# ototoi/pbrt-r3

Measured on AMD Instinct MI355X. Metric: Mrays/s, higher is better.
Workload: dtype f32

## Files before the change

### pbrt-r3_amd/csrc/pt_kernels.hip

```cpp
#include <hip/hip_runtime.h>
#include <cstdlib>
#include "pt_device.h"
#include "pt_device_math.h"
#include "pt_bxdf.h"
#include "pt_sphere.h"
#include "pt_texture.h"
#include <type_traits>
#include "pt_lobes.h"
#include "pt_kernels.h"
#include "../../include/pbrtgpu.h"

#ifndef PT_SHADE_PF_DEEP
#define PT_SHADE_PF_DEEP 0
#endif
#ifndef PT_LOBES_IN_LDS
#define PT_LOBES_IN_LDS 1
#endif
#ifndef PT_TEX_PROGS_GLOBAL
#define PT_TEX_PROGS_GLOBAL 1
#endif
#ifndef PT_LIGHTS_IN_LDS
#define PT_LIGHTS_IN_LDS 8
#endif
#ifndef PT_TEX_NOUNROLL
// ... 799 lines not shown
        "v_add_u32 %[sa], %[slot], %[sa]\n\t"
        "v_mov_b32 %[top], %[c0]\n\t"
        "ds_write_b32 %[sa], %[c0]\n\t"
        "s_mov_b64 exec, %[e1]\n\t"
        "v_add_u32 %[sa], %[slot], %[sa]\n\t"
        "v_mov_b32 %[top], %[c1]\n\t"
        "ds_write_b32 %[sa], %[c1]\n\t"
        "s_mov_b64 exec, %[e2]\n\t"
        "v_add_u32 %[sa], %[slot], %[sa]\n\t"
        "v_mov_b32 %[top], %[c2]\n\t"
        "ds_write_b32 %[sa], %[c2]\n\t"
        "s_mov_b64 exec, %[e3]\n\t"
        "v_add_u32 %[sa], %[slot], %[sa]\n\t"
        "v_mov_b32 %[top], %[c3]\n\t"
        "ds_write_b32 %[sa], %[c3]\n\t"
        "s_mov_b64 exec, %[sv]"
        : [sa] "+v"(sa), [top] "+v"(top), [sv] "=&s"(sv)
        : [e0] "s"(e0), [e1] "s"(e1), [e2] "s"(e2), [e3] "s"(e3), [c0] "v"(c0), [c1] "v"(c1), [c2] "v"(c2), [c3] "v"(c3), [slot] "s"(PT_SLOT)
        : "memory");
}
typedef __attribute__((address_space(3))) void* pt_lds_void;
typedef const __attribute__((address_space(1))) void* pt_global_cvoid;
typedef float pt_v4f __attribute__((ext_vector_type(4)));
typedef uint32_t pt_v4u __attribute__((ext_vector_type(4)));
PT_DEV float4 lds_load4(uint32_t a) { const pt_v4f v = *(__attribute__((address_space(3))) const pt_v4f*)(size_t)a; return make_float4(v.x, v.y, v.z, v.w); }
PT_DEV uint4 lds_load4u(uint32_t a) { const pt_v4u v = *(__attribute__((address_space(3))) const pt_v4u*)(size_t)a; return make_uint4(v.x, v.y, v.z, v.w); }
PT_DEV uint32_t node_round_issue(const PtScene& sc, LaneRay& r, TravCtx& c, bool w_node) {
    uint32_t ref = PT_EMPTY_REF, top = PT_EMPTY_REF;
    if (w_node) {
#ifdef PT_STACK_HIST
        atomicAdd(c.spill - ((size_t)blockIdx.x * PT_BLOCK + threadIdx.x) - PT_DIAG_WORDS + 1024u + min(fs_slot(c, r.sa), 63u), 1u);
#endif
        ref = r.top;
        r.sa -= PT_SLOT;
        top = lds_load(r.sa);
        c.n_nodes++;
    }
    lds_store(c.idx_pub, ref);
    __builtin_amdgcn_fence(__ATOMIC_RELEASE, "wavefront");
    __builtin_amdgcn_wave_barrier();
    __builtin_amdgcn_fence(__ATOMIC_ACQUIRE, "wavefront");
    {
        const uint4 ia = lds_load4u(c.idx_ld), ib = lds_load4u(c.idx_ld + 16u);
        const uint32_t ids[8] = {ia.x, ia.y, ia.z, ia.w, ib.x, ib.y, ib.z, ib.w};
        const uint32_t lane = threadIdx.x & 63u;
        const uint32_t coff = ((lane & 7u) ^ (lane >> 3)) << 4;
        const char* nb = reinterpret_cast<const char*>(sc.nodes);
        const uint32_t piece0 = (uint32_t)__builtin_amdgcn_readfirstlane((int)c.stage_wave);
#pragma unroll
        for (uint32_t j = 0; j < 8u; j++)
            if (ids[j] != PT_EMPTY_REF)
                __builtin_amdgcn_global_load_lds((pt_global_cvoid)(nb + ((ids[j] << 7) + coff)), (pt_lds_void)(size_t)(piece0 + j * 1024u), 16, 0, 0);
    }
    return top;
}
PT_DEV void node_round_finish(LaneRay& r, TravCtx& c, bool w_node, uint32_t top) {
    if (w_node) {
        const float4 nx = lds_load4(r.o_nx), fx = lds_load4(r.o_fx), ny = lds_load4(r.o_ny), fy = lds_load4(r.o_fy), nz = lds_load4(r.o_nz), fz = lds_load4(r.o_fz);
        const uint4 ch = lds_load4u(c.stage_chunk(6u));
        const uint32_t lut = lds_load(c.stage_chunk(7u) + 4u);
        const float ox = r.o.x, oy = r.o.y, oz = r.o.z, ix = r.idir.x, iy = r.idir.y, iz = r.idir.z;
#define PT_SLAB(C) (v_min3(v_min(r.tmax, (fx.C - ox) * ix), (fy.C - oy) * iy, (fz.C - oz) * iz) >= v_max3(v_max(r.tmin, (nx.C - ox) * ix), (ny.C - oy) * iy, (nz.C - oz) * iz))
        const bool h0 = PT_SLAB(x), h1 = PT_SLAB(y), h2 = PT_SLAB(z), h3 = PT_SLAB(w);
#undef PT_SLAB
        const bool T = (lut & r.m_t) != 0u, L = (lut & r.m_l) != 0u, R = (lut & r.m_r) != 0u;
        const uint32_t l0 = L ? ch.x : ch.y, l1 = L ? ch.y : ch.x, r0 = R ? ch.z : ch.w, r1 = R ? ch.w : ch.z;
        const uint32_t c0 = T ? l0 : r0, c1 = T ? l1 : r1, c2 = T ? r0 : l0, c3 = T ? r1 : l1;
        const unsigned long long H0 = __ballot(h0), H1 = __ballot(h1), H2 = __ballot(h2), H3 = __ballot(h3), Tm = __ballot(T), Lm = __ballot(L), Rm = __ballot(R);
        const unsigned long long yl = Lm & (H0 ^ H1), el0 = H1 ^ yl, el1 = H0 ^ yl;
        const unsigned long long yr = Rm & (H2 ^ H3), er0 = H3 ^ yr, er1 = H2 ^ yr;
        const unsigned long long y0 = Tm & (el0 ^ er0), e0 = er0 ^ y0, e2 = el0 ^ y0;
        const unsigned long long y1 = Tm & (el1 ^ er1), e1 = er1 ^ y1, e3 = el1 ^ y1;
        fs_push4_exec(r.sa, top, c0, c1, c2, c3, e0, e1, e2, e3);
        r.top = top;
    }
}

template <int TOUCH>
PT_DEV void node_step_lean(const PtScene& sc, LaneRay& r, TravCtx& c) {
    const uint32_t ref = r.top;
    r.sa -= PT_SLOT;
    uint32_t top = lds_load(r.sa);
    c.n_nodes++;
    const char* nb = reinterpret_cast<const char*>(sc.nodes);
    const uint32_t no = ref << 7;
    float4 nx, fx, ny, fy, nz, fz;
    uint4 ch;
#if PT_TOP_NODES > 0
    const bool in_lds = no < c.top_bytes;
    c.n_nodes_lds += in_lds ? 1u : 0u;
    if (in_lds) {
        const uint32_t la = c.top_lds + no - (no >> 3);
        nx = lds_load4(la + r.o_nx); fx = lds_load4(la + r.o_fx); ny = lds_load4(la + r.o_ny); fy = lds_load4(la + r.o_fy);
        nz = lds_load4(la + r.o_nz); fz = lds_load4(la + r.o_fz);
        ch = lds_load4u(la + 96u);
    }
    if (!in_lds)
#endif
    {
        nx = *reinterpret_cast<const float4*>(nb + (no + r.o_nx)); fx = *reinterpret_cast<const float4*>(nb + (no + r.o_fx));
        ny = *reinterpret_cast<const float4*>(nb + (no + r.o_ny)); fy = *reinterpret_cast<const float4*>(nb + (no + r.o_fy));
        nz = *reinterpret_cast<const float4*>(nb + (no + r.o_nz)); fz = *reinterpret_cast<const float4*>(nb + (no + r.o_fz));
        ch = *reinterpret_cast<const uint4*>(nb + (no + 96u));
    }
    const float ox = r.o.x, oy = r.o.y, oz = r.o.z, ix = r.idir.x, iy = r.idir.y, iz = r.idir.z;
#define PT_SLAB(C) (v_min3(v_min(r.tmax, (fx.C - ox) * ix), (fy.C - oy) * iy, (fz.C - oz) * iz) >= v_max3(v_max(r.tmin, (nx.C - ox) * ix), (ny.C - oy) * iy, (nz.C - oz) * iz))
    const bool h0 = PT_SLAB(x), h1 = PT_SLAB(y), h2 = PT_SLAB(z), h3 = PT_SLAB(w);
#undef PT_SLAB
    const bool T = __builtin_amdgcn_ubfe(r.sbits, __builtin_amdgcn_ubfe(ch.x, PT_REF_AXIS_SHIFT, 2), 1) != 0u;
    const bool L = __builtin_amdgcn_ubfe(r.sbits, __builtin_amdgcn_ubfe(ch.y, PT_REF_AXIS_SHIFT, 2), 1) != 0u;
    const bool R = __builtin_amdgcn_ubfe(r.sbits, __builtin_amdgcn_ubfe(ch.w, PT_REF_AXIS_SHIFT, 2), 1) != 0u;
    const uint32_t l0 = L ? ch.x : ch.y, l1 = L ? ch.y : ch.x, r0 = R ? ch.z : ch.w, r1 = R ? ch.w : ch.z;
    const uint32_t c0 = T ? l0 : r0, c1 = T ? l1 : r1, c2 = T ? r0 : l0, c3 = T ? r1 : l1;
    const unsigned long long H0 = __ballot(h0), H1 = __ballot(h1), H2 = __ballot(h2), H3 = __ballot(h3), Tm = __ballot(T), Lm = __ballot(L), Rm = __ballot(R);
    const unsigned long long yl = Lm & (H0 ^ H1), el0 = H1 ^ yl, el1 = H0 ^ yl;
    const unsigned long long yr = Rm & (H2 ^ H3), er0 = H3 ^ yr, er1 = H2 ^ yr;
    const unsigned long long y0 = Tm & (el0 ^ er0), e0 = er0 ^ y0, e2 = el0 ^ y0;
    const unsigned long long y1 = Tm & (el1 ^ er1), e1 = er1 ^ y1, e3 = el1 ^ y1;
    fs_push4_exec(r.sa, top, c0, c1, c2, c3, e0, e1, e2, e3);
    r.top = top;
    if constexpr (TOUCH != 0) {
        unsigned long long p0, p1, p2, p3 = 0ull;
        if (TOUCH >= 4) { p0 = e0; p1 = e1; p2 = e2; p3 = e3; }
        else { p0 = e0 & (e1 | e2 | e3); p1 = e1 & (e2 | e3); p2 = e2 & e3; }
        const unsigned long long me = 1ull << (threadIdx.x & 63u);
        const char* tb = reinterpret_cast<const char*>(sc.tris);
        auto touch = [&](uint32_t cref) {
            if (TOUCH == 2 && (cref & PT_LEAF_BIT)) return;
            if (TOUCH >= 3 && !(cref & PT_LEAF_BIT)) return;
            const char* a = (cref & PT_LEAF_BIT) ? tb + (size_t)(cref & PT_LEAF_FIRST_MASK) * 48u : nb + (size_t)(cref << 7);
            uint32_t v = *reinterpret_cast<const uint32_t*>(a);
            asm volatile("" :: "v"(v));
            if (TOUCH == 5 && ((cref >> PT_LEAF_COUNT_SHIFT) & 7u) >= 2u) {
                uint32_t w = *reinterpret_cast<const uint32_t*>(a + 128);
                asm volatile("" :: "v"(w));
            }
        };
        if (p0 & me) touch(c0);
        if (p1 & me) touch(c1);
        if (p2 & me) touch(c2);
        if (p3 & me) touch(c3);
    }
}

#ifndef PT_NODE_COOP
#define PT_NODE_COOP 1
#endif
#ifndef PT_COOP_TOUCH
#define PT_COOP_TOUCH 0
#endif
#if PT_NODE_COOP
#define PT_PAIR_U(x) ((uint32_t)__builtin_amdgcn_update_dpp(0, (int)(x), 0xB1, 0xF, 0xF, false))
#define PT_PAIR_F(x) __builtin_bit_cast(float, __builtin_amdgcn_update_dpp(0, __builtin_bit_cast(int, (x)), 0xB1, 0xF, 0xF, false))
template <int TOUCH>
PT_DEV void node_step_coop(const PtScene& sc, LaneRay& r, TravCtx& c, bool w_node, unsigned long long m_node) {
    constexpr unsigned long long kEven = 0x5555555555555555ull, kOdd = 0xAAAAAAAAAAAAAAAAull;
    const unsigned long long ev = m_node & kEven, od = m_node & kOdd;
    const unsigned long long m_y = ev | (ev << 1), m_z = od | (od >> 1);
    if (__builtin_amdgcn_inverse_ballot_w64(m_y | m_z)) {
        const uint32_t ref = r.top;
        const uint32_t no = ref << 7;
        const char* nb = reinterpret_cast<const char*>(sc.nodes);
        uint32_t top = PT_EMPTY_REF;
        const bool in_lds = w_node && no < c.top_bytes;
        if (w_node) { r.sa -= PT_SLOT; top = lds_load(r.sa); c.n_nodes++; c.n_nodes_lds += in_lds ? 1u : 0u; }
        const unsigned long long m_lds = __ballot(in_lds), le = m_lds & kEven, lo = m_lds & kOdd;
        const unsigned long long y_lds = le | (le << 1), z_lds = lo | (lo >> 1);
        const uint32_t base = in_lds ? c.top_lds + no - (no >> 3) : no;
        uint32_t a1 = base + r.o_nx, a2 = base + r.o_ny, a3 = base + r.o_nz;
        uint32_t b1 = PT_PAIR_U(base + r.o_fx), b2 = PT_PAIR_U(base + r.o_fy), b3 = PT_PAIR_U(base + r.o_fz);
        unsigned long long sv;
        asm volatile("s_mov_b64 %[sv], exec\n\ts_and_b64 exec, exec, %[om]\n\tv_swap_b32 %0, %3\n\tv_swap_b32 %1, %4\n\tv_swap_b32 %2, %5\n\ts_mov_b64 exec, %[sv]"
                     : "+v"(a1), "+v"(a2), "+v"(a3), "+v"(b1), "+v"(b2), "+v"(b3), [sv] "=&s"(sv) : [om] "s"(kOdd));
        float4 x1, x2, x3, x4, x5, x6;
        uint4 ch;
        if (__builtin_amdgcn_inverse_ballot_w64(m_y & y_lds)) { x1 = lds_load4(a1); x2 = lds_load4(a2); x3 = lds_load4(a3); }
        if (__builtin_amdgcn_inverse_ballot_w64(m_z & z_lds)) { x4 = lds_load4(b1); x5 = lds_load4(b2); x6 = lds_load4(b3); }
        if (in_lds) ch = lds_load4u(base + 96u);
        if (__builtin_amdgcn_inverse_ballot_w64(m_y & ~y_lds)) {
            x1 = *reinterpret_cast<const float4*>(nb + a1); x2 = *reinterpret_cast<const float4*>(nb + a2); x3 = *reinterpret_cast<const float4*>(nb + a3);
        }
        if (__builtin_amdgcn_inverse_ballot_w64(m_z & ~z_lds)) {
            x4 = *reinterpret_cast<const float4*>(nb + b1); x5 = *reinterpret_cast<const float4*>(nb + b2); x6 = *reinterpret_cast<const float4*>(nb + b3);
        }
        if (__builtin_amdgcn_inverse_ballot_w64(m_node & ~m_lds)) ch = *reinterpret_cast<const uint4*>(nb + (no + 96u));
        asm volatile("s_mov_b64 %[sv], exec\n\ts_and_b64 exec, exec, %[om]\n\t"
                     "v_swap_b32 %0, %12\n\tv_swap_b32 %1, %13\n\tv_swap_b32 %2, %14\n\tv_swap_b32 %3, %15\n\t"
                     "v_swap_b32 %4, %16\n\tv_swap_b32 %5, %17\n\tv_swap_b32 %6, %18\n\tv_swap_b32 %7, %19\n\t"
                     "v_swap_b32 %8, %20\n\tv_swap_b32 %9, %21\n\tv_swap_b32 %10, %22\n\tv_swap_b32 %11, %23\n\t"
                     "s_mov_b64 exec, %[sv]\n\ts_nop 1"
                     : "+v"(x1.x), "+v"(x1.y), "+v"(x1.z), "+v"(x1.w), "+v"(x2.x), "+v"(x2.y), "+v"(x2.z), "+v"(x2.w), "+v"(x3.x), "+v"(x3.y), "+v"(x3.z), "+v"(x3.w),
                       "+v"(x4.x), "+v"(x4.y), "+v"(x4.z), "+v"(x4.w), "+v"(x5.x), "+v"(x5.y), "+v"(x5.z), "+v"(x5.w), "+v"(x6.x), "+v"(x6.y), "+v"(x6.z), "+v"(x6.w), [sv] "=&s"(sv)
                     : [om] "s"(kOdd));
        const float ox = r.o.x, oy = r.o.y, oz = r.o.z, ix = r.idir.x, iy = r.idir.y, iz = r.idir.z;
#define PT_SLAB(C) (v_min3(v_min(r.tmax, (PT_PAIR_F(x4.C) - ox) * ix), (PT_PAIR_F(x5.C) - oy) * iy, (PT_PAIR_F(x6.C) - oz) * iz) >= \
                    v_max3(v_max(r.tmin, (x1.C - ox) * ix), (x2.C - oy) * iy, (x3.C - oz) * iz))
        const bool h0 = PT_SLAB(x), h1 = PT_SLAB(y), h2 = PT_SLAB(z), h3 = PT_SLAB(w);
#undef PT_SLAB
        const bool T = __builtin_amdgcn_ubfe(r.sbits, __builtin_amdgcn_ubfe(ch.x, PT_REF_AXIS_SHIFT, 2), 1) != 0u;
        const bool L = __builtin_amdgcn_ubfe(r.sbits, __builtin_amdgcn_ubfe(ch.y, PT_REF_AXIS_SHIFT, 2), 1) != 0u;
        const bool R = __builtin_amdgcn_ubfe(r.sbits, __builtin_amdgcn_ubfe(ch.w, PT_REF_AXIS_SHIFT, 2), 1) != 0u;
        const uint32_t l0 = L ? ch.x : ch.y, l1 = L ? ch.y : ch.x, r0 = R ? ch.z : ch.w, r1 = R ? ch.w : ch.z;
        const uint32_t c0 = T ? l0 : r0, c1 = T ? l1 : r1, c2 = T ? r0 : l0, c3 = T ? r1 : l1;
        const unsigned long long H0 = __ballot(h0) & m_node, H1 = __ballot(h1) & m_node, H2 = __ballot(h2) & m_node, H3 = __ballot(h3) & m_node;
        const unsigned long long Tm = __ballot(T), Lm = __ballot(L), Rm = __ballot(R);
        const unsigned long long yl = Lm & (H0 ^ H1), el0 = H1 ^ yl, el1 = H0 ^ yl;
        const unsigned long long yr = Rm & (H2 ^ H3), er0 = H3 ^ yr, er1 = H2 ^ yr;
        const unsigned long long y0 = Tm & (el0 ^ er0), e0 = er0 ^ y0, e2 = el0 ^ y0;
        const unsigned long long y1 = Tm & (el1 ^ er1), e1 = er1 ^ y1, e3 = el1 ^ y1;
        fs_push4_exec(r.sa, top, c0, c1, c2, c3, e0, e1, e2, e3);
        if (w_node) r.top = top;
        if constexpr (TOUCH != 0 && PT_COOP_TOUCH) {
            const unsigned long long p0 = e0 & (e1 | e2 | e3), p1 = e1 & (e2 | e3), p2 = e2 & e3;
            const char* tb = reinterpret_cast<const char*>(sc.tris);
            auto touch = [&](uint32_t cref) {
                if (!(cref & PT_LEAF_BIT)) return;
                uint32_t v = *reinterpret_cast<const uint32_t*>(tb + (size_t)(cref & PT_LEAF_FIRST_MASK) * 48u);
                asm volatile("" :: "v"(v));
            };
            if (__builtin_amdgcn_inverse_ballot_w64(p0)) touch(c0);
            if (__builtin_amdgcn_inverse_ballot_w64(p1)) touch(c1);
            if (__builtin_amdgcn_inverse_ballot_w64(p2)) touch(c2);
        }
    }
}
#endif

template <bool SPH, bool INST, bool ALPHA = false>
PT_DEV int32_t trace_closest(const PtScene& sc, V3 o, V3 d, float t_max, TravCtx& c, float* t_out, uint32_t* inst_out) {
    LaneRay r;
    ray_begin(sc, r, o, d, t_max);
    while (!ray_done(r)) ray_step<SPH, INST, ALPHA>(sc, r, false, c);
    *t_out = r.ray_tmax;
    *inst_out = r.best_inst;
    return r.best;
}
template <bool SPH, bool INST, bool ALPHA = false>
PT_DEV bool trace_any(const PtScene& sc, V3 o, V3 d, float t_max, TravCtx& c) {
    LaneRay r;
    ray_begin(sc, r, o, d, t_max);
    while (!ray_done(r)) ray_step<SPH, INST, ALPHA>(sc, r, true, c);
    return r.best >= 0;
}

PT_DEV void flush_counters(PtCounters* g, unsigned long long* s_cnt, unsigned long long regular, unsigned long long shadow,
                           unsigned long long nodes, unsigned long long tris) {
    if (threadIdx.x < 4) s_cnt[threadIdx.x] = 0;
    __syncthreads();
    if (regular) atomicAdd(&s_cnt[0], regular);
    if (shadow) atomicAdd(&s_cnt[1], shadow);
    if (nodes) atomicAdd(&s_cnt[2], nodes);
    if (tris) atomicAdd(&s_cnt[3], tris);
    __syncthreads();
    if (threadIdx.x == 0) {
        if (s_cnt[0]) atomicAdd(&g->regular_rays, s_cnt[0]);
        if (s_cnt[1]) atomicAdd(&g->shadow_rays, s_cnt[1]);
        if (s_cnt[2]) atomicAdd(&g->nodes, s_cnt[2]);
        if (s_cnt[3]) atomicAdd(&g->tris, s_cnt[3]);
    }
}

PT_DEV uint32_t wave_ticket(uint32_t* ticket) {
    uint32_t base = 0;
    if ((threadIdx.x & 63) == 0) base = atomicAdd(ticket, 64u);
    return (uint32_t)__builtin_amdgcn_readfirstlane((int)base);
}

#ifdef PT_PROFILE_PHASES
#define PT_PROF_T(name) const unsigned long long name = (unsigned long long)__builtin_readcyclecounter()
#define PT_PROF_SET(name) name = (unsigned long long)__builtin_readcyclecounter()
#else
#define PT_PROF_T(name) do { } while (0)
#define PT_PROF_SET(name) do { } while (0)
#endif
#ifndef PT_REFILL_MIN
#define PT_REFILL_MIN 8
#endif
#ifndef PT_LEAF_MIN
#define PT_LEAF_MIN 24
#endif
#ifndef PT_LEAF_MIN_INST
#define PT_LEAF_MIN_INST 40
#endif
#ifndef PT_TRACE_WAVES
#define PT_TRACE_WAVES 4
#endif
#ifndef PT_TRACE_DIST_WAVES
#if PT_NODE_STAGED
#define PT_TRACE_DIST_WAVES 3
#else
#define PT_TRACE_DIST_WAVES 4
#endif
#endif

#ifndef PT_LEAF_TRIS_MIN
#define PT_LEAF_TRIS_MIN 56
#endif
#ifndef PT_LEAF_LANES_MIN
#define PT_LEAF_LANES_MIN 18
#endif
#ifndef PT_WALK_BATCH
#define PT_WALK_BATCH 1
#endif
#ifndef PT_SPH_LANES_MIN
#define PT_SPH_LANES_MIN 8
#endif
#ifndef PT_LEAF_TRIS_FUSED
#define PT_LEAF_TRIS_FUSED 0
#endif
template <bool DIST, bool SPH, bool INST = false, int TOUCH = 0, bool ALPHA = false>
PT_DEV void trace_body(const PtScene& sc, const PtPaths& P, const PtQueues& Q, PtCounters* cnt, uint32_t* spill, uint32_t spill_depth, uint32_t* err) {
    constexpr uint32_t TB = DIST ? PT_TBLOCK : PT_BLOCK;
    __shared__ uint32_t s_stack[(DIST ? PT_FS_SLOTS : PT_LDS_STACK) * TB];
    __shared__ unsigned long long s_cnt[4];
#if PT_NODE_STAGED
    __shared__ __attribute__((aligned(16))) unsigned char s_stage[DIST ? (PT_BLOCK / 64) * 8192 : 16];
    __shared__ uint32_t s_idx[DIST ? PT_BLOCK + PT_BLOCK / 4 : 1];
    float4* const s_res = reinterpret_cast<float4*>(s_stage + (threadIdx.x >> 6) * 8192u) - (threadIdx.x & ~63u);
    unsigned char* const s_map = reinterpret_cast<unsigned char*>(&s_idx[(threadIdx.x >> 6) * 80u + 64u]) - (threadIdx.x & ~63u);
#else
    __shared__ float4 s_res[DIST ? TB : 1];
    __shared__ unsigned char s_map[DIST ? TB : 1];
#endif
#if PT_TOP_NODES > 0 && !PT_NODE_STAGED
    __shared__ float4 s_top[DIST ? PT_TOP_NODES * 7 : 1];
#endif
    TravCtx c;
    c.lds = &s_stack[threadIdx.x];
    c.top_lds = 0; c.top_bytes = 0; c.n_nodes_lds = 0;
    c.spill_stride = gridDim.x * TB;
    c.spill = spill + PT_DIAG_WORDS + (size_t)blockIdx.x * TB + threadIdx.x;
    c.spill_depth = spill_depth;
    c.n_nodes = 0; c.n_tris = 0; c.overflow = 0;
    c.lane_base = 0; c.stage_wave = 0; c.stage_own = 0; c.idx_pub = 0; c.idx_ld = 0;
    if constexpr (DIST) {
        s_stack[threadIdx.x] = PT_EMPTY_REF;
        c.lane_base = lds_addr_of(&s_stack[threadIdx.x]);
#if PT_NODE_STAGED
        const uint32_t ln = threadIdx.x & 63u, wv = threadIdx.x >> 6;
        c.stage_wave = lds_addr_of(reinterpret_cast<const uint32_t*>(s_stage + wv * 8192u));
        c.stage_own = c.stage_wave + (ln >> 3) * 1024u + (ln & 7u) * 128u;
        c.idx_pub = lds_addr_of(&s_idx[wv * 80u + (ln & 7u) * 8u + (ln >> 3)]);
        c.idx_ld = lds_addr_of(&s_idx[wv * 80u + (ln >> 3) * 8u]);
#endif
    }
#if PT_TOP_NODES > 0 && !PT_NODE_STAGED
    if constexpr (DIST) {
        const uint32_t n_top = min(sc.n_top, (uint32_t)PT_TOP_NODES);
        const float4* src = reinterpret_cast<const float4*>(sc.nodes);
        for (uint32_t k = threadIdx.x; k < n_top * 7u; k += TB) { const uint32_t nd = k / 7u; s_top[k] = src[nd * 8u + (k - nd * 7u)]; }
        c.top_lds = lds_addr_of(reinterpret_cast<const uint32_t*>(s_top));
        c.top_bytes = n_top << 7;
        __syncthreads();
    }
#endif
    const uint32_t n_cur = Q.counts[PT_Q_CUR], n_sh = Q.counts[PT_Q_SHADOW], n_pr = Q.counts[PT_Q_PROBE];
    const uint32_t total = n_cur + n_sh + n_pr;
    const uint32_t lane = threadIdx.x & 63;
    const unsigned long long below = (lane == 0) ? 0ull : (~0ull >> (64 - lane));
    unsigned long long regular = 0, shadow = 0;

    int kind = 0;
    uint32_t p = 0;
    LaneRay r;
    r.sp = 0;
    r.sa = c.lane_base; r.sa_limit = 0;
    r.top = PT_EMPTY_REF;
    bool more = total > 0;
    bool sph_wait = false;
    int pf_stage = 0, pf_kind = 0;
    uint32_t pf_raw = 0, pf_count = 0, pf_used = 0, pf_p = 0;
    uint32_t seg = blockIdx.x & 7u, seg_dry = 0;
    const uint32_t seg_len = (((total + 7u) >> 3) + 63u) & ~63u;
    float4 pf_o = make_float4(0.0f, 0.0f, 0.0f, 0.0f), pf_d = pf_o;
#ifdef PT_PROFILE_PHASES
    unsigned long long prof[16] = {0, 0, 0, 0, 0, 0, 0, 0, 0, 0, 0, 0, 0, 0, 0, 0};
    long long prof_t0 = __builtin_readcyclecounter();
#endif
    for (;;) {
#ifdef PT_PROFILE_PHASES
        long long pt_iter = __builtin_readcyclecounter();
#endif
        if (pf_stage == 0) {
            if (more) {
                if (lane == 0) pf_raw = atomicAdd(&Q.counts[PT_Q_SEG_TICKET0 + 32u * seg], 64u);
                pf_stage = 1;
            }
        } else if (pf_stage == 1) {
            const uint32_t seg_lo = seg * seg_len, seg_hi = min(total, seg_lo + seg_len);
            const uint32_t base = seg_lo + (uint32_t)__builtin_amdgcn_readfirstlane((int)pf_raw);
            if (seg_lo >= total || base >= seg_hi) {
                seg = (seg + 1u) & 7u;
                if (++seg_dry == 8u) more = false;
                pf_stage = 0;
            } else {
                seg_dry = 0;
                pf_count = min(64u, seg_hi - base);
                pf_used = 0;
                const uint32_t item = base + lane;
                if (lane < pf_count) {
                    if (item < n_cur) { pf_p = Q.cur[item]; pf_kind = 1; }
                    else if (item < n_cur + n_sh) { pf_p = Q.shadow[item - n_cur]; pf_kind = 2; }
                    else { pf_p = Q.probe[item - n_cur - n_sh]; pf_kind = 3; }
                }
                pf_stage = 2;
            }
        } else if (pf_stage == 2) {
            if (lane < pf_count) {
                const float4* so = pf_kind == 1 ? P.ray_o : (pf_kind == 2 ? P.sh_o : P.pr_o);
                const float4* sd = pf_kind == 1 ? P.ray_d : (pf_kind == 2 ? P.sh_d : P.pr_d);
                pf_o = so[pf_p]; pf_d = sd[pf_p];
            }
            pf_stage = 3;
        }
#ifdef PT_PROFILE_PHASES
        const long long pt_pf = __builtin_readcyclecounter();
        prof[14] += (unsigned long long)(pt_pf - pt_iter);
#endif
        if (kind != 0 && ray_done(r)) {
            if (kind == 1) { P.hit_t[p] = r.ray_tmax; P.hit_rec[p] = r.best; if (INST && (!ALPHA || sc.n_instances)) P.hit_inst[p] = r.best_inst; }
            else if (kind == 2) P.occluded[p] = r.best >= 0 ? 1 : 0;
            else P.probe_rec[p] = r.best;
            kind = 0;
        }
        {
            const unsigned long long idle = __ballot(kind == 0);
            const uint32_t n_idle = (uint32_t)__popcll(idle);
            if (pf_stage == 3 && (n_idle >= PT_REFILL_MIN || idle == ~0ull || (!more && n_idle != 0))) {
                const uint32_t take = min(n_idle, pf_count - pf_used);
                const uint32_t rank = (uint32_t)__popcll(idle & below);
                const int src = (int)((pf_used + rank) & 63u);
                const uint32_t np = (uint32_t)__shfl((int)pf_p, src, 64);
                const int nk = __shfl(pf_kind, src, 64);
                float4 ro, rd;
                ro.x = __shfl(pf_o.x, src, 64); ro.y = __shfl(pf_o.y, src, 64); ro.z = __shfl(pf_o.z, src, 64); ro.w = __shfl(pf_o.w, src, 64);
                rd.x = __shfl(pf_d.x, src, 64); rd.y = __shfl(pf_d.y, src, 64); rd.z = __shfl(pf_d.z, src, 64);
                if (kind == 0 && rank < take) {
                    p = np; kind = nk;
                    if (nk == 2) shadow++; else regular++;
                    if constexpr (DIST) ray_begin_fs(sc, r, c, f4_3(ro), mk3(rd.x, rd.y, rd.z), ro.w);
                    else ray_begin(sc, r, f4_3(ro), mk3(rd.x, rd.y, rd.z), ro.w);
                }
                pf_used += take;
                if (pf_used == pf_count) pf_stage = 0;
            }
        }
#ifdef PT_PROFILE_PHASES
        prof[15] += (unsigned long long)(__builtin_readcyclecounter() - pt_pf);
#endif
        if (__ballot(kind != 0) == 0) {
            if (!more && pf_stage == 0) break;
            continue;
        }
        bool w_tri = kind != 0 && ray_wants_tri(r);
        bool w_node = kind != 0 && ray_wants_node(r);
        unsigned long long m_tri = __ballot(w_tri), m_node = __ballot(w_node);
#ifdef PT_PROFILE_PHASES
        long long pt0 = __builtin_readcyclecounter();
        prof[10] += (unsigned long long)(pt0 - pt_iter);
#endif
        if constexpr (DIST) {
            constexpr bool SPHDEF = SPH && !PT_NODE_STAGED && PT_LEAF_LANES_MIN > 0;
            bool sround = SPH && !SPHDEF;
            unsigned long long m_tri_s = 0;
            if constexpr (SPHDEF) {
                m_tri_s = __ballot(w_tri && sph_wait);
                m_tri &= ~m_tri_s;
            }
            const bool sph_go = SPHDEF && (uint32_t)__popcll(m_tri_s) >= (uint32_t)PT_SPH_LANES_MIN;
            const uint32_t tcnt = w_tri ? ((r.top >> PT_LEAF_COUNT_SHIFT) & 7u) + 1u : 0u;
            uint32_t tcnt_r = tcnt;
            bool w_serve = w_tri;
#if PT_LEAF_LANES_MIN > 0
            unsigned long long c0 = 0, c1 = 0, c2 = 0, c3 = 0;
            const uint32_t n_parked = (sph_go || (uint32_t)__popcll(m_tri) >= (uint32_t)PT_LEAF_LANES_MIN) ? (uint32_t)PT_LEAF_TRIS_MIN : 0u;
#else
            const unsigned long long c0 = __ballot((tcnt & 1u) != 0), c1 = __ballot((tcnt & 2u) != 0), c2 = __ballot((tcnt & 4u) != 0),
                                     c3 = __ballot((tcnt & 8u) != 0);
            const uint32_t n_parked = (uint32_t)(__popcll(c0) + 2 * __popcll(c1) + 4 * __popcll(c2) + 8 * __popcll(c3));
#endif
            const uint32_t wbase = threadIdx.x & ~63u;
            uint32_t lf_pre = 0, lf_items = 0;
            bool lf_served = false, lf_valid = false;
            int lf_kk = 0;
            float lf_tmax = PT_INF;
            RayPre lf_rp;
            TriVerts lf_tv;
            auto leaf_issue = [&](auto sr_tag) {
                constexpr bool SR = decltype(sr_tag)::value;
                (void)SR;
#if PT_LEAF_LANES_MIN > 0
                c0 = __ballot((tcnt_r & 1u) != 0); c1 = __ballot((tcnt_r & 2u) != 0); c2 = __ballot((tcnt_r & 4u) != 0); c3 = __ballot((tcnt_r & 8u) != 0);
#endif
                lf_pre = (uint32_t)(__popcll(c0 & below) + 2 * __popcll(c1 & below) + 4 * __popcll(c2 & below) + 8 * __popcll(c3 & below));
                lf_served = w_serve && lf_pre + tcnt_r <= 64u;
                const unsigned long long m_served = __ballot(lf_served);
                const int last = 63 - __clzll(m_served);
                lf_items = (uint32_t)__shfl((int)(lf_pre + tcnt_r), last, 64);
                if (lf_served)
                    for (uint32_t k = 0; k < tcnt_r; k++) s_map[wbase + lf_pre + k] = (unsigned char)lane;
                __builtin_amdgcn_fence(__ATOMIC_RELEASE, "wavefront");
                __builtin_amdgcn_wave_barrier();
                __builtin_amdgcn_fence(__ATOMIC_ACQUIRE, "wavefront");
                lf_valid = lane < lf_items;
                const int o = lf_valid ? (int)s_map[wbase + lane] : 0;
                const uint32_t k = lane - (uint32_t)__shfl((int)lf_pre, o, 64);
                const uint32_t first = (uint32_t)__shfl((int)(r.top & PT_LEAF_FIRST_MASK), o, 64);
                lf_rp.o = mk3(__shfl(r.rp.o.x, o, 64), __shfl(r.rp.o.y, o, 64), __shfl(r.rp.o.z, o, 64));
                lf_rp.d = mk3(0.0f, 0.0f, 0.0f);
                if ((SPH && SR) || sc.any_one_sided) lf_rp.d = mk3(__shfl(r.rp.d.x, o, 64), __shfl(r.rp.d.y, o, 64), __shfl(r.rp.d.z, o, 64));
                if constexpr (SPH && SR) lf_tmax = __shfl(r.ray_tmax, o, 64);
                lf_kk = __shfl(r.rp.kx | (r.rp.ky << 2) | (r.rp.kz << 4) | ((kind == 2 ? 1 : 0) << 6), o, 64);
                lf_rp.kx = lf_kk & 3; lf_rp.ky = (lf_kk >> 2) & 3; lf_rp.kz = (lf_kk >> 4) & 3;
                lf_rp.sx = __shfl(r.rp.sx, o, 64); lf_rp.sy = __shfl(r.rp.sy, o, 64); lf_rp.sz = __shfl(r.rp.sz, o, 64);
                lf_rp.dperm = lf_rp.d;
                lf_tv.p0 = lf_rp.d; lf_tv.p1 = lf_rp.d; lf_tv.p2 = lf_rp.d; lf_tv.prim = 0; lf_tv.flags = 0;
                if (lf_valid) lf_tv = load_tri(sc.tris, first + k);
            };
            auto leaf_finish = [&](auto sr_tag) {
                constexpr bool SR = decltype(sr_tag)::value;
                (void)SR;
                bool sphere_rec = false;
                if constexpr (SPH) sphere_rec = lf_valid && (lf_tv.flags & PT_TRI_SPHERE) != 0;
                unsigned long long m_sitems = 0;
                if constexpr (SPHDEF && !SR) { m_sitems = __ballot(sphere_rec); }
                if (lf_valid) {
                    TriCore tc;
                    const bool tri_ok = tri_core(lf_rp, lf_tv.p0, lf_tv.p1, lf_tv.p2, lf_tv.flags, tc);
                    float4 res = make_float4(tri_ok ? 1.0f : 0.0f, tc.t_scaled, tc.det, tc.t);
                    if (SR && sphere_rec) {
                        SphHit sh;
                        sh.t = 0.0f; sh.a_hi = 0.0f; sh.b_hi = 0.0f;
                        const bool ok = sph_hit_test_inl(sc.spheres[__float_as_uint(lf_tv.p0.x)], lf_rp.o, lf_rp.d, lf_tmax, (lf_kk & 64) ? 2.0f * PT_PI : PT_PI, &sh);
                        res = make_float4(ok ? 2.0f : 0.0f, sh.a_hi, sh.b_hi, sh.t);
                    }
                    s_res[wbase + lane] = res;
                }
                __builtin_amdgcn_fence(__ATOMIC_RELEASE, "wavefront");
                __builtin_amdgcn_wave_barrier();
                __builtin_amdgcn_fence(__ATOMIC_ACQUIRE, "wavefront");
                bool walk = lf_served;
                if constexpr (SPHDEF) {
                    if (!SR && lf_served && ((m_sitems >> lf_pre) & ((1ull << tcnt_r) - 1ull)) != 0ull) { sph_wait = true; walk = false; }
                    if (SR && lf_served) sph_wait = false;
                }
                if (walk) {
                    const uint32_t rec0 = fs_pop(c, r.sa, r.top) & PT_LEAF_FIRST_MASK;
                    const bool any_hit = kind == 2;
                    bool leaf_hit = false;
                    uint32_t tested = tcnt;
#if PT_WALK_BATCH
                    bool stop = false;
                    for (uint32_t k0 = 0; k0 < tcnt && !stop; k0 += 4u) {
                        const uint32_t b = wbase + lf_pre + k0;
                        const float4 va = s_res[b], vb = s_res[wbase + min(lf_pre + k0 + 1u, 63u)], vc = s_res[wbase + min(lf_pre + k0 + 2u, 63u)],
                                     vd = s_res[wbase + min(lf_pre + k0 + 3u, 63u)];
                        auto step = [&](const float4 v, uint32_t k) {
                            if (stop || k >= tcnt) return;
                            bool acc;
                            if (SPH && SR && v.x == 2.0f) acc = !(v.y > r.ray_tmax) && !(v.z > r.ray_tmax);
                            else acc = v.x != 0.0f && tri_accept(v.y, v.z, r.ray_tmax);
                            if (acc) {
                                r.best = (int32_t)(rec0 + k); leaf_hit = true;
                                if (any_hit) { r.sa = c.lane_base; r.top = PT_EMPTY_REF; tested = k + 1; stop = true; return; }
                                r.ray_tmax = v.w;
                            }
                        };
                        step(va, k0); step(vb, k0 + 1u); step(vc, k0 + 2u); step(vd, k0 + 3u);
                    }
#else
                    for (uint32_t k = 0; k < tcnt; k++) {
                        const float4 v = s_res[wbase + lf_pre + k];
                        bool acc;
                        if (SPH && SR && v.x == 2.0f) acc = !(v.y > r.ray_tmax) && !(v.z > r.ray_tmax);
                        else acc = v.x != 0.0f && tri_accept(v.y, v.z, r.ray_tmax);
                        if (acc) {
                            r.best = (int32_t)(rec0 + k); leaf_hit = true;
                            if (any_hit) { r.sa = c.lane_base; r.top = PT_EMPTY_REF; tested = k + 1; break; }
                            r.ray_tmax = v.w;
                        }
                    }
#endif
                    c.n_tris += tested;
                    if (leaf_hit && !any_hit) r.tmax = r.ray_tmax;
                }
            };
#ifdef PT_FORCE_GENERAL_VISIT
            const bool lean = false;
#elif defined(PT_EXP_NO_GENERAL_VISIT)
            const bool lean = true;
#else
            const bool lean = __ballot(w_node && r.sa >= r.sa_limit) == 0ull;
#endif
#if !PT_NODE_STAGED
            if (lean && m_node != 0 && n_parked < PT_LEAF_TRIS_MIN) {
                PT_PROF_T(t0);
#if PT_NODE_COOP
                if constexpr (TOUCH != 0 || PT_NODE_COOP == 2) node_step_coop<TOUCH>(sc, r, c, w_node, m_node);
                else if (w_node) node_step_lean<TOUCH>(sc, r, c);
#else
                if (w_node) node_step_lean<TOUCH>(sc, r, c);
#endif
                PT_PROF_T(t1);
#ifdef PT_PROFILE_PHASES
                prof[2] += t1 - t0; prof[3] += 1; prof[4] += (unsigned long long)__popcll(m_node);
#endif
#else
            if (lean) {
                const bool do_node = m_node != 0 && (PT_LEAF_TRIS_FUSED > 0 || n_parked < PT_LEAF_TRIS_MIN);
                const bool do_leaf = m_tri != 0 && (!do_node || (PT_LEAF_TRIS_FUSED > 0 && n_parked >= PT_LEAF_TRIS_FUSED));
                (void)do_leaf;
#if PT_LEAF_TRIS_FUSED > 0
                uint32_t below_top = PT_EMPTY_REF;
                PT_PROF_T(t0);
                if (do_node) below_top = node_round_issue(sc, r, c, w_node);
                PT_PROF_T(t1);
                if (do_leaf) leaf_issue(std::integral_constant<bool, SPH>{});
                PT_PROF_T(t2);
                asm volatile("s_waitcnt vmcnt(0)" ::: "memory");
                __builtin_amdgcn_wave_barrier();
                PT_PROF_T(t3);
                if (do_node) node_round_finish(r, c, w_node, below_top);
                PT_PROF_T(t4);
                if (do_leaf) leaf_finish(std::integral_constant<bool, SPH>{});
                PT_PROF_T(t5);
#else
                unsigned long long t0 = 0, t1 = 0, t2 = 0, t3 = 0, t4 = 0, t5 = 0;
                (void)t0; (void)t1; (void)t2; (void)t3; (void)t4; (void)t5;
                PT_PROF_SET(t0);
                if (do_node) {
                    const uint32_t below_top = node_round_issue(sc, r, c, w_node);
                    PT_PROF_SET(t1); PT_PROF_SET(t2);
                    asm volatile("s_waitcnt vmcnt(0)" ::: "memory");
                    __builtin_amdgcn_wave_barrier();
                    PT_PROF_SET(t3);
                    node_round_finish(r, c, w_node, below_top);
                    PT_PROF_SET(t4); PT_PROF_SET(t5);
                } else {
                    PT_PROF_SET(t1);
                    leaf_issue(std::integral_constant<bool, SPH>{});
                    PT_PROF_SET(t2);
#ifdef PT_PROFILE_PHASES
                    asm volatile("s_waitcnt vmcnt(0)" ::: "memory");
#endif
                    PT_PROF_SET(t3); PT_PROF_SET(t4);
                    leaf_finish(std::integral_constant<bool, SPH>{});
                    PT_PROF_SET(t5);
                }
#endif
#ifdef PT_PROFILE_PHASES
                if (do_node) { prof[0] += t1 - t0; prof[2] += t4 - t3; prof[3] += 1; prof[4] += (unsigned long long)__popcll(m_node); }
                if (do_leaf) { prof[5] += t2 - t1; prof[7] += t5 - t4; prof[8] += 1; prof[9] += (unsigned long long)lf_items; }
                prof[do_node ? 1 : 6] += t3 - t2;
#endif
#endif
            } else if (m_node != 0 && n_parked < PT_LEAF_TRIS_MIN) {
                PT_PROF_T(t0);
                if (w_node) node_step_general(sc, r, c);
                PT_PROF_T(t1);
#ifdef PT_PROFILE_PHASES
                prof[12] += t1 - t0; prof[13] += 1; prof[4] += (unsigned long long)__popcll(m_node);
#endif
            } else if ((m_tri | m_tri_s) != 0) {
                if constexpr (SPHDEF) {
                    sround = sph_go || m_tri == 0;
                    w_serve = w_tri && (sph_wait == sround);
                    tcnt_r = w_serve ? tcnt : 0u;
                }
                PT_PROF_T(t0);
                if (SPHDEF && sround) leaf_issue(std::true_type{}); else leaf_issue(std::integral_constant<bool, SPH && !SPHDEF>{});
#ifdef PT_PROFILE_PHASES
                PT_PROF_T(t0b);
                asm volatile("s_waitcnt vmcnt(0)" ::: "memory");
                PT_PROF_T(t0c);
                prof[5] += t0b - t0; prof[6] += t0c - t0b;
#endif
                if (SPHDEF && sround) leaf_finish(std::true_type{}); else leaf_finish(std::integral_constant<bool, SPH && !SPHDEF>{});
                PT_PROF_T(t1);
#ifdef PT_PROFILE_PHASES
                prof[7] += t1 - t0c; prof[8] += 1; prof[9] += (unsigned long long)lf_items;
#endif
            }
        } else {
        if (m_node != 0 && __popcll(m_tri) < (INST ? PT_LEAF_MIN_INST : PT_LEAF_MIN)) {
            if (w_node) ray_step_node(sc, r, c);
#ifdef PT_PROFILE_PHASES
            prof[12] += (unsigned long long)(__builtin_readcyclecounter() - pt0); prof[13] += 1; prof[4] += (unsigned long long)__popcll(m_node);
#endif
        } else {
            if constexpr (INST) {
                if (w_tri) {
                    if (r.top == PT_INST_EXIT_REF) {
                        (void)stk_pop(c, r.top, r.sp);
                        const float w_tmax = __uint_as_float(stk_pop(c, r.top, r.sp)), w_tmin = __uint_as_float(stk_pop(c, r.top, r.sp));
                        const float4 ro = (kind == 1 ? P.ray_o : (kind == 2 ? P.sh_o : P.pr_o))[p], rd = (kind == 1 ? P.ray_d : (kind == 2 ? P.sh_d : P.pr_d))[p];
                        const bool hit_inside = r.best >= 0 && r.best_inst == r.cur_inst;
                        ray_set_direction_state(r, f4_3(ro), mk3(rd.x, rd.y, rd.z));
                        r.tmin = w_tmin; r.tmax = hit_inside ? r.ray_tmax : w_tmax;
                        r.cur_inst = 0;
                    } else ray_step_tri_enter<SPH, ALPHA>(sc, r, kind == 2, c);
                }
            } else {
                if (w_tri) ray_step_tri<SPH, INST>(sc, r, kind == 2, c);
            }
#ifdef PT_PROFILE_PHASES
            prof[7] += (unsigned long long)(__builtin_readcyclecounter() - pt0); prof[8] += 1; prof[9] += (unsigned long long)__popcll(m_tri);
#endif
        }
        }
    }
#ifdef PT_PROFILE_PHASES
    prof[11] = (unsigned long long)(__builtin_readcyclecounter() - prof_t0);
    if (lane == 0) for (int i = 0; i < 16; i++) atomicAdd(reinterpret_cast<unsigned long long*>(spill) + i, prof[i]);
#endif
    if (c.overflow) atomicOr(err, 1u);
    flush_counters(cnt, s_cnt, regular, shadow, c.n_nodes, c.n_tris);
    {
        unsigned long long v = c.n_nodes_lds;
        for (int o = 32; o > 0; o >>= 1) v += (unsigned long long)__shfl_xor((int)(v >> 32), o, 64) << 32 | (unsigned int)__shfl_xor((int)(unsigned int)v, o, 64);
        if ((threadIdx.x & 63) == 0 && v) atomicAdd(&cnt->nodes_lds, v);
    }
}
extern "C" __global__ void __launch_bounds__(PT_TBLOCK, PT_TRACE_DIST_WAVES) k_trace(PtScene sc, PtPaths P, PtQueues Q, PtCounters* cnt, uint32_t* spill,
                                                              uint32_t spill_depth, uint32_t* err) {
    trace_body<true, false>(sc, P, Q, cnt, spill, spill_depth, err);
}
extern "C" __global__ void __launch_bounds__(PT_TBLOCK, PT_TRACE_DIST_WAVES) k_trace_far(PtScene sc, PtPaths P, PtQueues Q, PtCounters* cnt, uint32_t* spill,
                                                                   uint32_t spill_depth, uint32_t* err) {
    trace_body<true, false, false, PT_TOUCH_VARIANT>(sc, P, Q, cnt, spill, spill_depth, err);
}
extern "C" __global__ void __launch_bounds__(PT_BLOCK, PT_TRACE_WAVES) k_trace_seq(PtScene sc, PtPaths P, PtQueues Q, PtCounters* cnt, uint32_t* spill,
                                                                  uint32_t spill_depth, uint32_t* err) {
    trace_body<false, false>(sc, P, Q, cnt, spill, spill_depth, err);
}
#ifndef PT_TRACE_INST_WAVES
#define PT_TRACE_INST_WAVES 3
#endif

extern "C" __global__ void __launch_bounds__(PT_BLOCK, PT_TRACE_INST_WAVES) k_trace_inst(PtScene sc, PtPaths P, PtQueues Q, PtCounters* cnt, uint32_t* spill,
                                                                       uint32_t spill_depth, uint32_t* err) {
    trace_body<false, true, true>(sc, P, Q, cnt, spill, spill_depth, err);
}
extern "C" __global__ void __launch_bounds__(PT_BLOCK, PT_TRACE_INST_WAVES) k_trace_alpha(PtScene sc, PtPaths P, PtQueues Q, PtCounters* cnt, uint32_t* spill,
                                                                        uint32_t spill_depth, uint32_t* err) {
    trace_body<false, true, true, 0, true>(sc, P, Q, cnt, spill, spill_depth, err);
}
extern "C" __global__ void __launch_bounds__(PT_TBLOCK, PT_TRACE_DIST_WAVES) k_trace_sph_dist(PtScene sc, PtPaths P, PtQueues Q, PtCounters* cnt, uint32_t* spill,
                                                                           uint32_t spill_depth, uint32_t* err) {
    trace_body<true, true>(sc, P, Q, cnt, spill, spill_depth, err);
}
extern "C" __global__ void __launch_bounds__(PT_BLOCK, 2) k_trace_sph(PtScene sc, PtPaths P, PtQueues Q, PtCounters* cnt, uint32_t* spill,
                                                                      uint32_t spill_depth, uint32_t* err) {
    trace_body<false, true>(sc, P, Q, cnt, spill, spill_depth, err);
}

template <bool SPH, bool INST = false, bool ALPHA = false>
PT_DEV void trace_batch_body(const PtScene& sc, uint32_t n, const float* o, const float* d, const float* tmax, pt_hit* out, uint8_t* occ_out, int any_hit,
                             uint32_t* ticket, PtCounters* cnt, uint32_t* spill, uint32_t spill_depth, uint32_t* err) {
    __shared__ uint32_t s_stack[PT_LDS_STACK * PT_BLOCK];
    __shared__ unsigned long long s_cnt[4];
    TravCtx c;
    c.lds = &s_stack[threadIdx.x];
    c.spill_stride = gridDim.x * PT_BLOCK;
    c.spill = spill + PT_DIAG_WORDS + (size_t)blockIdx.x * PT_BLOCK + threadIdx.x;
    c.spill_depth = spill_depth;
    c.n_nodes = 0; c.n_tris = 0; c.overflow = 0;
    unsigned long long regular = 0, shadow = 0;
    for (;;) {
        uint32_t base = wave_ticket(ticket);
        if (base >= n) break;
        uint32_t i = base + (threadIdx.x & 63);
        if (i >= n) continue;
        V3 ro = ld3(o + 3 * (size_t)i), rd = ld3(d + 3 * (size_t)i);
        if (any_hit) {
            shadow++;
            occ_out[i] = trace_any<SPH, INST, ALPHA>(sc, ro, rd, tmax[i], c) ? 1 : 0;
        } else {
            regular++;
            float t;
            uint32_t inst = 0;
            int32_t rec = trace_closest<SPH, INST, ALPHA>(sc, ro, rd, tmax[i], c, &t, &inst);
            pt_hit h;
            h.t = 0.0f; h.prim = -1; h.b0 = 0.0f; h.b1 = 0.0f;
            if (rec >= 0 && INST && inst) {
                h.t = t; h.prim = (int32_t)sc.instances[inst - 1u].world_prim;
            } else if (rec >= 0) {
                TriVerts tv = load_tri(sc.tris, (uint32_t)rec);
                h.t = t; h.prim = (int32_t)tv.prim;
                if (!(SPH && (tv.flags & PT_TRI_SPHERE))) {
                    RayPre rp;
                    ray_precompute(rp, ro, rd);
                    TriHit th;
                    tri_test(rp, tv.p0, tv.p1, tv.p2, tv.flags, PT_INF, th);
                    h.b0 = th.b0; h.b1 = th.b1;
                }
            }
            out[i] = h;
        }
    }
    if (c.overflow) atomicOr(err, 1u);
    flush_counters(cnt, s_cnt, regular, shadow, c.n_nodes, c.n_tris);
}
extern "C" __global__ void __launch_bounds__(PT_BLOCK) k_trace_batch(PtScene sc, uint32_t n, const float* o, const float* d, const float* tmax,
                                                                    pt_hit* out, uint8_t* occ_out, int any_hit, uint32_t* ticket, PtCounters* cnt,
                                                                    uint32_t* spill, uint32_t spill_depth, uint32_t* err) {
    trace_batch_body<false>(sc, n, o, d, tmax, out, occ_out, any_hit, ticket, cnt, spill, spill_depth, err);
}
extern "C" __global__ void __launch_bounds__(PT_BLOCK) k_trace_batch_sph(PtScene sc, uint32_t n, const float* o, const float* d, const float* tmax,
                                                                        pt_hit* out, uint8_t* occ_out, int any_hit, uint32_t* ticket, PtCounters* cnt,
                                                                        uint32_t* spill, uint32_t spill_depth, uint32_t* err) {
    trace_batch_body<true>(sc, n, o, d, tmax, out, occ_out, any_hit, ticket, cnt, spill, spill_depth, err);
}
extern "C" __global__ void __launch_bounds__(PT_BLOCK) k_trace_batch_inst(PtScene sc, uint32_t n, const float* o, const float* d, const float* tmax,
                                                                         pt_hit* out, uint8_t* occ_out, int any_hit, uint32_t* ticket, PtCounters* cnt,
                                                                         uint32_t* spill, uint32_t spill_depth, uint32_t* err) {
    trace_batch_body<true, true>(sc, n, o, d, tmax, out, occ_out, any_hit, ticket, cnt, spill, spill_depth, err);
}
extern "C" __global__ void __launch_bounds__(PT_BLOCK) k_trace_batch_alpha(PtScene sc, uint32_t n, const float* o, const float* d, const float* tmax,
                                                                          pt_hit* out, uint8_t* occ_out, int any_hit, uint32_t* ticket, PtCounters* cnt,
                                                                          uint32_t* spill, uint32_t spill_depth, uint32_t* err) {
    trace_batch_body<true, true, true>(sc, n, o, d, tmax, out, occ_out, any_hit, ticket, cnt, spill, spill_depth, err);
}

extern "C" __global__ void __launch_bounds__(PT_BLOCK) k_wavefront_results(PtScene sc, PtPaths P, uint32_t n, const uint8_t* kind, pt_hit* out, uint8_t* occ) {
    for (uint32_t i = blockIdx.x * blockDim.x + threadIdx.x; i < n; i += gridDim.x * blockDim.x) {
        const uint32_t k = kind[i];
        pt_hit h;
        h.t = 0.0f; h.prim = -1; h.b0 = 0.0f; h.b1 = 0.0f;
        uint8_t oc = 0;
        if (k == 2u) oc = P.occluded[i];
        else {
            const int32_t rec = k == 1u ? P.hit_rec[i] : P.probe_rec[i];
            if (rec >= 0) {
                const uint32_t inst = (k == 1u && sc.n_instances) ? P.hit_inst[i] : 0u;
                TriVerts tv = load_tri(sc.tris, (uint32_t)rec);
                h.prim = inst ? (int32_t)sc.instances[inst - 1u].world_prim : (int32_t)tv.prim;
                if (k == 1u) {
                    h.t = P.hit_t[i];
                    if (!inst && !(tv.flags & (PT_TRI_SPHERE | PT_TRI_INSTANCE))) {
                        RayPre rp;
                        ray_precompute(rp, f4_3(P.ray_o[i]), f4_3(P.ray_d[i]));
                        TriHit th;
                        tri_test(rp, tv.p0, tv.p1, tv.p2, tv.flags, PT_INF, th);
                        h.b0 = th.b0; h.b1 = th.b1;
                    }
                }
            }
        }
        out[i] = h;
        occ[i] = oc;
    }
}
hipError_t ptk_wavefront_results(hipStream_t st, int grid, const PtScene& sc, const PtPaths& P, uint32_t n, const uint8_t* kind, pt_hit* out, uint8_t* occ) {
    hipLaunchKernelGGL(k_wavefront_results, dim3(grid), dim3(PT_BLOCK), 0, st, sc, P, n, kind, out, occ);
    return hipGetLastError();
}

extern "C" __global__ void __launch_bounds__(PT_BLOCK) k_expand_tiles(const int4* tiles, const uint32_t* tile_off, uint32_t n_tiles, int32_t sb_x0, int32_t sb_y0,
                                                                     uint32_t sb_w, uint32_t* pixels, uint32_t* bitmap, uint32_t* err) {
    for (uint32_t t = blockIdx.x; t < n_tiles; t += gridDim.x) {
        const int4 tl = tiles[t];
        const uint32_t w = (uint32_t)(tl.z - tl.x), n = w * (uint32_t)(tl.w - tl.y), off = tile_off[t];
        for (uint32_t i = threadIdx.x; i < n; i += blockDim.x) {
            const uint32_t x = (uint32_t)(tl.x - sb_x0) + i % w, y = (uint32_t)(tl.y - sb_y0) + i / w;
            pixels[off + i] = x | (y << 16);
            const uint32_t bit = y * sb_w + x;
            if (atomicOr(&bitmap[bit >> 5], 1u << (bit & 31u)) & (1u << (bit & 31u))) atomicOr(err, 2u);
        }
    }
}
hipError_t ptk_expand_tiles(hipStream_t st, const int4* tiles, const uint32_t* tile_off, uint32_t n_tiles, int32_t sb_x0, int32_t sb_y0, uint32_t sb_w,
                            uint32_t* pixels, uint32_t* bitmap, uint32_t* err) {
    hipLaunchKernelGGL(k_expand_tiles, dim3(n_tiles < 4096u ? n_tiles : 4096u), dim3(PT_BLOCK), 0, st, tiles, tile_off, n_tiles, sb_x0, sb_y0, sb_w, pixels, bitmap, err);
    return hipGetLastError();
}

extern "C" __global__ void __launch_bounds__(PT_BLOCK) k_gen(PtScene sc, PtPaths P, PtQueues Q, const uint32_t* pixels, uint32_t n_pix,
                                                            uint32_t s0, uint32_t n_samples, PtCounters* cnt) {
    uint32_t n = n_pix * n_samples;
    for (uint32_t i = blockIdx.x * blockDim.x + threadIdx.x; i < n; i += gridDim.x * blockDim.x) {
        uint32_t pk = pixels[i % n_pix];
        uint32_t s = s0 + i / n_pix;
        int32_t rx = (int32_t)(pk & 0xffffu), ry = (int32_t)(pk >> 16);
        int32_t px = rx + sc.film.sample_bounds[0], py = ry + sc.film.sample_bounds[1];
        Sampler sm;
// ... 2534 lines not shown
```

Measured before the change: 1104.

## Pre-filter leaf hits in helper lanes and defer ray retirement to handout

Helper lanes that test triangles for a leaf now also run the accept test against the owning ray's current tmax. They write results to LDS only for candidate hits and publish a candidate ballot, so the owning lane walks only the candidate bits instead of every triangle in the leaf. Separately, in the distributed trace path, finished rays are no longer written back every iteration. They are retired only when a refill hands out new work or when no more work remains, which cuts scattered global stores and divergent branches per iteration. The cost is an extra shuffle of tmax, an extra ballot, and later result writes; the first-candidate shortcut relies on a stale tmax staying conservative.

Measured after the change: 1148, median of 6. 1.04x the previous value.

```diff
diff --git a/pbrt-r3_amd/csrc/pt_kernels.hip b/pbrt-r3_amd/csrc/pt_kernels.hip
--- a/pbrt-r3_amd/csrc/pt_kernels.hip
+++ b/pbrt-r3_amd/csrc/pt_kernels.hip
@@ -1125,6 +1125,12 @@
 #ifndef PT_WALK_BATCH
 #define PT_WALK_BATCH 1
 #endif
+#ifndef PT_LEAF_HELPER_ACCEPT
+#define PT_LEAF_HELPER_ACCEPT 1
+#endif
+#ifndef PT_RETIRE_AT_HANDOUT
+#define PT_RETIRE_AT_HANDOUT 1
+#endif
 #ifndef PT_SPH_LANES_MIN
 #define PT_SPH_LANES_MIN 8
 #endif
@@ -1240,16 +1246,24 @@
         const long long pt_pf = __builtin_readcyclecounter();
         prof[14] += (unsigned long long)(pt_pf - pt_iter);
 #endif
-        if (kind != 0 && ray_done(r)) {
-            if (kind == 1) { P.hit_t[p] = r.ray_tmax; P.hit_rec[p] = r.best; if (INST && (!ALPHA || sc.n_instances)) P.hit_inst[p] = r.best_inst; }
-            else if (kind == 2) P.occluded[p] = r.best >= 0 ? 1 : 0;
-            else P.probe_rec[p] = r.best;
-            kind = 0;
+        constexpr bool LATE_RETIRE = DIST && PT_RETIRE_AT_HANDOUT;
+#define PT_RETIRE()                                                                                                                                      \
+        if (kind != 0 && ray_done(r)) {                                                                                                                  \
+            if (kind == 1) { P.hit_t[p] = r.ray_tmax; P.hit_rec[p] = r.best; if (INST && (!ALPHA || sc.n_instances)) P.hit_inst[p] = r.best_inst; }      \
+            else if (kind == 2) P.occluded[p] = r.best >= 0 ? 1 : 0;                                                                                     \
+            else P.probe_rec[p] = r.best;                                                                                                                \
+            kind = 0;                                                                                                                                    \
+        }
+        if constexpr (LATE_RETIRE) {
+            if (!more) { PT_RETIRE() }
+        } else {
+            PT_RETIRE()
         }
         {
-            const unsigned long long idle = __ballot(kind == 0);
+            const unsigned long long idle = LATE_RETIRE ? __ballot(kind == 0 || ray_done(r)) : __ballot(kind == 0);
             const uint32_t n_idle = (uint32_t)__popcll(idle);
             if (pf_stage == 3 && (n_idle >= PT_REFILL_MIN || idle == ~0ull || (!more && n_idle != 0))) {
+                if constexpr (LATE_RETIRE) { PT_RETIRE() }
                 const uint32_t take = min(n_idle, pf_count - pf_used);
                 const uint32_t rank = (uint32_t)__popcll(idle & below);
                 const int src = (int)((pf_used + rank) & 63u);
@@ -1268,10 +1282,11 @@
                 if (pf_used == pf_count) pf_stage = 0;
             }
         }
+#undef PT_RETIRE
 #ifdef PT_PROFILE_PHASES
         prof[15] += (unsigned long long)(__builtin_readcyclecounter() - pt_pf);
 #endif
-        if (__ballot(kind != 0) == 0) {
+        if ((LATE_RETIRE ? __ballot(kind != 0 && !ray_done(r)) : __ballot(kind != 0)) == 0) {
             if (!more && pf_stage == 0) break;
             continue;
         }
@@ -1303,6 +1318,7 @@
             const uint32_t n_parked = (uint32_t)(__popcll(c0) + 2 * __popcll(c1) + 4 * __popcll(c2) + 8 * __popcll(c3));
 #endif
             const uint32_t wbase = threadIdx.x & ~63u;
+            constexpr bool HACC = PT_LEAF_HELPER_ACCEPT == 2 || (PT_LEAF_HELPER_ACCEPT == 1 && !SPH);
             uint32_t lf_pre = 0, lf_items = 0;
             bool lf_served = false, lf_valid = false;
             int lf_kk = 0;
@@ -1332,7 +1348,7 @@
                 lf_rp.o = mk3(__shfl(r.rp.o.x, o, 64), __shfl(r.rp.o.y, o, 64), __shfl(r.rp.o.z, o, 64));
                 lf_rp.d = mk3(0.0f, 0.0f, 0.0f);
                 if ((SPH && SR) || sc.any_one_sided) lf_rp.d = mk3(__shfl(r.rp.d.x, o, 64), __shfl(r.rp.d.y, o, 64), __shfl(r.rp.d.z, o, 64));
-                if constexpr (SPH && SR) lf_tmax = __shfl(r.ray_tmax, o, 64);
+                if constexpr ((SPH && SR) || HACC) lf_tmax = __shfl(r.ray_tmax, o, 64);
                 lf_kk = __shfl(r.rp.kx | (r.rp.ky << 2) | (r.rp.kz << 4) | ((kind == 2 ? 1 : 0) << 6), o, 64);
                 lf_rp.kx = lf_kk & 3; lf_rp.ky = (lf_kk >> 2) & 3; lf_rp.kz = (lf_kk >> 4) & 3;
                 lf_rp.sx = __shfl(r.rp.sx, o, 64); lf_rp.sy = __shfl(r.rp.sy, o, 64); lf_rp.sz = __shfl(r.rp.sz, o, 64);
@@ -1347,18 +1363,23 @@
                 if constexpr (SPH) sphere_rec = lf_valid && (lf_tv.flags & PT_TRI_SPHERE) != 0;
                 unsigned long long m_sitems = 0;
                 if constexpr (SPHDEF && !SR) { m_sitems = __ballot(sphere_rec); }
+                bool cand = false;
                 if (lf_valid) {
                     TriCore tc;
                     const bool tri_ok = tri_core(lf_rp, lf_tv.p0, lf_tv.p1, lf_tv.p2, lf_tv.flags, tc);
                     float4 res = make_float4(tri_ok ? 1.0f : 0.0f, tc.t_scaled, tc.det, tc.t);
+                    if constexpr (HACC) cand = tri_ok && tri_accept(tc.t_scaled, tc.det, lf_tmax);
                     if (SR && sphere_rec) {
                         SphHit sh;
                         sh.t = 0.0f; sh.a_hi = 0.0f; sh.b_hi = 0.0f;
                         const bool ok = sph_hit_test_inl(sc.spheres[__float_as_uint(lf_tv.p0.x)], lf_rp.o, lf_rp.d, lf_tmax, (lf_kk & 64) ? 2.0f * PT_PI : PT_PI, &sh);
                         res = make_float4(ok ? 2.0f : 0.0f, sh.a_hi, sh.b_hi, sh.t);
+                        cand = ok;
                     }
-                    s_res[wbase + lane] = res;
+                    if (!HACC || cand) s_res[wbase + lane] = res;
                 }
+                const unsigned long long m_cand = HACC ? __ballot(cand) : 0ull;
+                (void)m_cand;
                 __builtin_amdgcn_fence(__ATOMIC_RELEASE, "wavefront");
                 __builtin_amdgcn_wave_barrier();
                 __builtin_amdgcn_fence(__ATOMIC_ACQUIRE, "wavefront");
@@ -1372,6 +1393,24 @@
                     const bool any_hit = kind == 2;
                     bool leaf_hit = false;
                     uint32_t tested = tcnt;
+                    if constexpr (HACC) {
+                    uint32_t bits = (uint32_t)(m_cand >> lf_pre) & ((1u << tcnt) - 1u);
+                    bool first = true;
+                    while (bits != 0u) {
+                        const uint32_t k = (uint32_t)__builtin_ctz(bits);
+                        bits &= bits - 1u;
+                        const float4 v = s_res[wbase + lf_pre + k];
+                        bool acc;
+                        if (SPH && SR && v.x == 2.0f) acc = !(v.y > r.ray_tmax) && !(v.z > r.ray_tmax);
+                        else acc = first || tri_accept(v.y, v.z, r.ray_tmax);
+                        first = false;
+                        if (acc) {
+                            r.best = (int32_t)(rec0 + k); leaf_hit = true;
+                            if (any_hit) { r.sa = c.lane_base; r.top = PT_EMPTY_REF; tested = k + 1u; break; }
+                            r.ray_tmax = v.w;
+                        }
+                    }
+                    } else {
 #if PT_WALK_BATCH
                     bool stop = false;
                     for (uint32_t k0 = 0; k0 < tcnt && !stop; k0 += 4u) {
@@ -1404,6 +1443,7 @@
                         }
                     }
 #endif
+                    }
                     c.n_tris += tested;
                     if (leaf_hit && !any_hit) r.tmax = r.ray_tmax;
                 }
```
